# bentotten/radiation_ppo

Measured on AMD Instinct MI355X. Metric: env steps/sec (whole node) at 4096 envs; PPO iters/sec at 1/2/4/8 GPUs, higher is better.
Workload: dtype f32 policy / f64+int32 env

## Files before the change

### include/radsearch.h

```cpp
#ifndef RADSEARCH_H
#define RADSEARCH_H

#include <stddef.h>
#include <stdint.h>

#ifdef __cplusplus
extern "C" {
#endif

#define RS_ABI_VERSION 4
#define RS_OBS_DIM 11
#define RS_NUM_ACTIONS 9
#define RS_MAX_AGENTS 8
#define RS_MAX_OBS 7

typedef void* rs_stream_t;
typedef struct rs_handle rs_handle;

enum {
    RS_OK = 0,
    RS_ERR_INVALID_ARG = 1,
    RS_ERR_HIP = 2,
    RS_ERR_WORKSPACE = 3,
    RS_ERR_UNSUPPORTED = 4
// ... 55 lines not shown

int rs_poisson_probe(const double* lam, const uint32_t* t, const uint32_t* episode, const uint32_t* env_id, int64_t count, uint32_t seed,
                     int64_t* serial, int64_t* group3, int64_t* group4, int32_t* candidates, rs_stream_t stream);

int rs_error_flags(rs_handle* h, rs_stream_t stream, uint32_t* flags_out);

int rs_gae(const float* rew, const float* val, const uint8_t* cut, const float* last_val, float* adv, float* ret,
           int32_t T, int32_t M, double gamma, double lam, rs_stream_t stream);

size_t rs_ppo_prepare_workspace_bytes(int32_t N);
int rs_ppo_prepare(const uint8_t* cut, const float* adv, float* w, float* adv_n, float* mean_std, void* workspace, int32_t T, int32_t N,
                   int32_t n_total, rs_stream_t stream);

typedef struct rs_mlp_params {
    const float *w1, *b1, *w2, *b2, *w3, *b3;
} rs_mlp_params;

int rs_policy_forward(const rs_mlp_params* actor, const rs_mlp_params* critic, const float* x, int32_t M,
                      float* logits, float* value, rs_stream_t stream);

int rs_ff_team_step(const rs_mlp_params* actors, const rs_mlp_params* critics, int32_t num_agents, const float* x, const float* u,
                    int64_t* act, float* logp_val_boot, int8_t* act8, const uint8_t* mask, int32_t num_envs, rs_stream_t stream);

typedef struct rs_rollout_args {
    int32_t steps_per_epoch;
    int32_t steps_per_episode;
    float* obs;
    int64_t* act;
    float* logp;
    float* val;
    float* rew;
    float* last_val;
    uint8_t* cut;
    float* source_tar;
    float* cur_obs;
    double* w_count;
    double* w_mean;
    double* w_sq;
    double* w_std;
    int32_t* steps_in_ep;
    float* ep_ret;
    int32_t* done_count;
    int32_t* oob_count;
    double* ep_ret_sum;
    double* ep_len_sum;
    int32_t* ep_count;
    double* ep_ret_sq_sum;
    float* ep_ret_max;
    float* ep_ret_min;
} rs_rollout_args;

int rs_rollout(rs_handle* h, const rs_mlp_params* actor, const rs_mlp_params* critic, const rs_rollout_args* args,
               rs_stream_t stream);

typedef struct rs_ppo_batch {
    const float* x;
    const int64_t* act;
    const float* adv;
    const float* ret;
    const float* logp_old;
    const float* w;
    int32_t M;
    float clip_ratio, alpha, vf_coef;
} rs_ppo_batch;

size_t rs_ppo_grad_workspace_bytes(void);
#define RS_PPO_STATS_TAIL 16
#define RS_PPO_GRAD_FLOATS (10441 + RS_PPO_STATS_TAIL)
int rs_ppo_grad(const rs_mlp_params* actor, const rs_mlp_params* critic, const rs_ppo_batch* batch, float* grads,
                double* stats, void* workspace, const int32_t* stop_flag, rs_stream_t stream);

typedef struct rs_update_state {
    int32_t adam_step;
    int32_t stopped;
    int32_t iters;
    int32_t pad;
    double last_stats[5];
} rs_update_state;

int rs_adam_step(const rs_mlp_params* actor, const rs_mlp_params* critic, const float* grads, float* m, float* v,
                 const double* stats, rs_update_state* state, float lr, float kl_threshold, rs_stream_t stream);

int rs_ppo_update_step(const rs_mlp_params* actor, const rs_mlp_params* critic, const rs_ppo_batch* batch, float* grads,
                       double* stats, void* workspace, float* m, float* v, rs_update_state* state, float lr, float kl_threshold,
                       rs_stream_t stream);

typedef struct rs_maps rs_maps;
enum {
    RS_MAPERR_RING_FULL = 1,
    RS_MAPERR_VISIT_OVERFLOW = 2,
    RS_MAPERR_OFF_MAP = 4
};
size_t rs_maps_state_bytes(int32_t num_envs, int32_t num_agents, int32_t steps_per_episode, int32_t map_x, int32_t map_y);
int rs_maps_create(int32_t num_envs, int32_t num_agents, int32_t steps_per_episode, int32_t map_x, int32_t map_y,
                   double resolution_accuracy, const float* visit_table, void* workspace, size_t workspace_bytes,
                   rs_stream_t stream, rs_maps** out);
void rs_maps_destroy(rs_maps* m);
int rs_maps_reset(rs_maps* m, const uint8_t* mask, rs_stream_t stream);
int rs_maps_update(rs_maps* m, rs_handle* env, const float* obs, const float* pred, const uint8_t* mask, rs_stream_t stream);
int rs_maps_stack(rs_maps* m, float* actor_stack, float* critic_stack, rs_stream_t stream);
int rs_maps_field(rs_maps* m, const char* name, void** dev_ptr, int32_t* elem_bytes, int32_t* rows, int32_t* cols);

int32_t rs_cnn_trunk_slab_row(int32_t in_channels);
int32_t rs_cnn_trunk_slab_rows(int64_t num_samples, int32_t in_channels);
int32_t rs_cnn_trunk_scratch_floats(int32_t in_channels);
int rs_cnn_trunk_forward(const float* maps, const int64_t* cells, const int64_t* pcells, int32_t num_agents, int32_t agent,
// ... 259 lines not shown
```

### radiation_ppo_amd/_lib.py

```python
import ctypes as C
import os

import torch

_PKG = os.path.dirname(os.path.abspath(__file__))
LIB_PATH = os.environ.get("RS_LIB_PATH") or os.path.join(_PKG, "lib", "librs_hip.so")

RS_OBS_DIM = 11
RS_MAX_AGENTS = 8
RS_MAX_OBS = 7

ENVERR_ZERO_DIST = 1
ENVERR_IDLE_STALL = 2
ENVERR_CORRECT_CAP = 4
ENVERR_BAD_ACTION = 8
ENVERR_NO_PATH = 16

MAPERR_RING_FULL = 1
MAPERR_VISIT_OVERFLOW = 2
MAPERR_OFF_MAP = 4


class RsConfig(C.Structure):
    _fields_ = [
# ... 32 lines not shown
class RsMlpParams(C.Structure):
    _fields_ = [(n, C.c_void_p) for n in ("w1", "b1", "w2", "b2", "w3", "b3")]


class RsCnnHeadParams(C.Structure):
    _fields_ = [(n, C.c_void_p) for n in ("w1", "b1", "w2", "b2", "w3", "b3")]


class RsCnnConvParams(C.Structure):
    _fields_ = [(n, C.c_void_p) for n in ("w1", "b1", "w2", "b2")]


class RsRolloutArgs(C.Structure):
    _fields_ = [("steps_per_epoch", C.c_int32), ("steps_per_episode", C.c_int32)] + [
        (n, C.c_void_p) for n in ("obs", "act", "logp", "val", "rew", "last_val", "cut", "source_tar", "cur_obs", "w_count",
                                  "w_mean", "w_sq", "w_std", "steps_in_ep", "ep_ret", "done_count", "oob_count",
                                  "ep_ret_sum", "ep_len_sum", "ep_count", "ep_ret_sq_sum", "ep_ret_max", "ep_ret_min")]


class RsPpoBatch(C.Structure):
    _fields_ = [("x", C.c_void_p), ("act", C.c_void_p), ("adv", C.c_void_p), ("ret", C.c_void_p), ("logp_old", C.c_void_p),
                ("w", C.c_void_p), ("M", C.c_int32), ("clip_ratio", C.c_float), ("alpha", C.c_float), ("vf_coef", C.c_float)]


class RsInfo(C.Structure):
    _fields_ = [("out_of_bounds", C.c_void_p), ("out_of_bounds_count", C.c_void_p), ("blocked", C.c_void_p),
                ("collision", C.c_void_p)]


SYMBOLS = [
    ("rs_strerror", C.c_char_p, [C.c_int]),
    ("rs_abi_version", C.c_int, []),
    ("rs_state_bytes", C.c_size_t, [C.POINTER(RsConfig)]),
    ("rs_create", C.c_int, [C.POINTER(RsConfig), C.c_void_p, C.c_size_t, C.c_void_p, C.POINTER(C.c_void_p)]),
    ("rs_destroy", None, [C.c_void_p]),
    ("rs_state_field", C.c_int, [C.c_void_p, C.c_char_p, C.POINTER(C.c_void_p), C.POINTER(C.c_int32),
                                 C.POINTER(C.c_int32), C.POINTER(C.c_int32)]),
    ("rs_set_epoch_end", C.c_int, [C.c_void_p, C.c_void_p]),
    ("rs_reset", C.c_int, [C.c_void_p, C.c_void_p, C.c_void_p, C.c_void_p, C.c_void_p, C.c_void_p,
                           C.POINTER(RsInfo), C.c_void_p]),
    ("rs_refresh", C.c_int, [C.c_void_p, C.c_void_p, C.c_void_p, C.c_void_p, C.c_void_p, C.c_void_p, C.c_void_p, C.c_void_p,
                             C.c_void_p, C.c_void_p, C.c_void_p, C.c_void_p, C.POINTER(RsInfo), C.c_void_p]),
    ("rs_step", C.c_int, [C.c_void_p, C.c_void_p, C.c_void_p, C.c_void_p, C.c_void_p, C.c_void_p,
                          C.POINTER(RsInfo), C.c_void_p]),
    ("rs_action_uniforms", C.c_int, [C.c_void_p, C.c_void_p, C.c_void_p]),
    ("rs_poisson_probe", C.c_int, [C.c_void_p, C.c_void_p, C.c_void_p, C.c_void_p, C.c_int64, C.c_uint32, C.c_void_p, C.c_void_p,
                                   C.c_void_p, C.c_void_p, C.c_void_p]),
    ("rs_error_flags", C.c_int, [C.c_void_p, C.c_void_p, C.POINTER(C.c_uint32)]),
    ("rs_policy_forward", C.c_int, [C.POINTER(RsMlpParams), C.POINTER(RsMlpParams), C.c_void_p, C.c_int32, C.c_void_p,
                                    C.c_void_p, C.c_void_p]),
    ("rs_ff_team_step", C.c_int, [C.POINTER(RsMlpParams), C.POINTER(RsMlpParams), C.c_int32, C.c_void_p, C.c_void_p, C.c_void_p,
                                  C.c_void_p, C.c_void_p, C.c_void_p, C.c_int32, C.c_void_p]),
    ("rs_rollout", C.c_int, [C.c_void_p, C.POINTER(RsMlpParams), C.POINTER(RsMlpParams), C.POINTER(RsRolloutArgs), C.c_void_p]),
    ("rs_ppo_grad_workspace_bytes", C.c_size_t, []),
    ("rs_ppo_grad", C.c_int, [C.POINTER(RsMlpParams), C.POINTER(RsMlpParams), C.POINTER(RsPpoBatch), C.c_void_p, C.c_void_p,
                              C.c_void_p, C.c_void_p, C.c_void_p]),
    ("rs_adam_step", C.c_int, [C.POINTER(RsMlpParams), C.POINTER(RsMlpParams), C.c_void_p, C.c_void_p, C.c_void_p, C.c_void_p,
                               C.c_void_p, C.c_float, C.c_float, C.c_void_p]),
    ("rs_ppo_update_step", C.c_int, [C.POINTER(RsMlpParams), C.POINTER(RsMlpParams), C.POINTER(RsPpoBatch), C.c_void_p, C.c_void_p,
                                     C.c_void_p, C.c_void_p, C.c_void_p, C.c_void_p, C.c_float, C.c_float, C.c_void_p]),
    ("rs_maps_state_bytes", C.c_size_t, [C.c_int32, C.c_int32, C.c_int32, C.c_int32, C.c_int32]),
    ("rs_maps_create", C.c_int, [C.c_int32, C.c_int32, C.c_int32, C.c_int32, C.c_int32, C.c_double, C.c_void_p, C.c_void_p,
                                 C.c_size_t, C.c_void_p, C.POINTER(C.c_void_p)]),
    ("rs_maps_destroy", None, [C.c_void_p]),
    ("rs_maps_reset", C.c_int, [C.c_void_p, C.c_void_p, C.c_void_p]),
    ("rs_maps_update", C.c_int, [C.c_void_p, C.c_void_p, C.c_void_p, C.c_void_p, C.c_void_p, C.c_void_p]),
    ("rs_maps_stack", C.c_int, [C.c_void_p, C.c_void_p, C.c_void_p, C.c_void_p]),
    ("rs_maps_field", C.c_int, [C.c_void_p, C.c_char_p, C.POINTER(C.c_void_p), C.POINTER(C.c_int32), C.POINTER(C.c_int32),
                                C.POINTER(C.c_int32)]),
    ("rs_cnn_trunk_slab_row", C.c_int32, [C.c_int32]),
    ("rs_cnn_trunk_slab_rows", C.c_int32, [C.c_int64, C.c_int32]),
    ("rs_cnn_trunk_scratch_floats", C.c_int32, [C.c_int32]),
    ("rs_cnn_trunk_forward", C.c_int, [C.c_void_p, C.c_void_p, C.c_void_p, C.c_int32, C.c_int32, C.c_int64, C.c_void_p, C.c_void_p,
                                       C.c_void_p, C.c_void_p, C.c_void_p, C.c_void_p, C.c_void_p, C.c_void_p, C.c_void_p, C.c_void_p]),
    ("rs_cnn_trunk_backward", C.c_int, [C.c_void_p, C.c_void_p, C.c_void_p, C.c_int32, C.c_int32, C.c_int64, C.c_void_p, C.c_void_p,
                                        C.c_void_p, C.c_void_p, C.c_void_p, C.c_void_p, C.c_void_p, C.c_void_p]),
    ("rs_gae", C.c_int, [C.c_void_p, C.c_void_p, C.c_void_p, C.c_void_p, C.c_void_p, C.c_void_p, C.c_int32,
                         C.c_int32, C.c_double, C.c_double, C.c_void_p]),
    ("rs_ppo_prepare_workspace_bytes", C.c_size_t, [C.c_int32]),
    ("rs_ppo_prepare", C.c_int, [C.c_void_p] * 6 + [C.c_int32, C.c_int32, C.c_int32, C.c_void_p]),
    ("rs_pfgru_step", C.c_int, [C.c_void_p, C.c_void_p, C.c_void_p, C.c_void_p, C.c_void_p, C.c_void_p, C.c_void_p, C.c_void_p,
                                C.c_int32, C.c_double, C.c_void_p, C.c_int32, C.c_int32, C.c_void_p]),
    ("rs_pfgru_step_recorded", C.c_int, [C.c_void_p] * 7 + [C.c_int32, C.c_double, C.c_void_p, C.c_int32, C.c_int32, C.c_void_p]),
    ("rs_pfgru_pass", C.c_int, [C.c_void_p] * 7 + [C.c_double, C.c_void_p, C.c_void_p, C.c_int32, C.c_int32, C.c_void_p]),
    ("rs_pfgru_reset", C.c_int, [C.c_void_p, C.c_void_p, C.c_void_p, C.c_void_p, C.c_void_p, C.c_void_p, C.c_int32, C.c_int32,
                                 C.c_void_p]),
    ("rs_pfgru_sized_weight_floats", C.c_int32, [C.c_int32]),
    ("rs_pfgru_sized_step", C.c_int, [C.c_void_p] * 8 + [C.c_int32, C.c_double, C.c_void_p, C.c_int32, C.c_int32, C.c_int32, C.c_void_p]),
    ("rs_pfgru_sized_pass", C.c_int, [C.c_void_p] * 7 + [C.c_double, C.c_void_p, C.c_void_p, C.c_int32, C.c_int32, C.c_int32, C.c_void_p]),
    ("rs_pfgru_sized_step_recorded", C.c_int, [C.c_void_p] * 7 + [C.c_int32, C.c_double, C.c_void_p, C.c_int32, C.c_int32, C.c_int32,
                                                                    C.c_void_p]),
    ("rs_pfgru_sized_reset", C.c_int, [C.c_void_p] * 6 + [C.c_int32, C.c_int32, C.c_int32, C.c_void_p]),
    ("rs_pfgru_draws", C.c_int, [C.c_void_p, C.c_int32, C.c_int32, C.c_void_p, C.c_void_p, C.c_void_p, C.c_void_p]),
    ("rs_pfgru_train", C.c_int, [C.c_void_p] * 15 + [C.c_int32, C.c_int32, C.c_double, C.c_double, C.c_double, C.c_double, C.c_void_p]),
    ("rs_pfgru_train_keyed", C.c_int, [C.c_void_p] * 14 + [C.c_int32, C.c_int32, C.c_double, C.c_double, C.c_double, C.c_double, C.c_void_p]),
    ("rs_pfgru_sized_train_weight_floats", C.c_int32, [C.c_int32]),
    ("rs_pfgru_sized_train_grad_floats", C.c_int32, [C.c_int32]),
    ("rs_pfgru_sized_draws", C.c_int, [C.c_void_p, C.c_int32, C.c_int32, C.c_int32, C.c_void_p, C.c_void_p, C.c_void_p, C.c_void_p]),
    ("rs_pfgru_sized_train", C.c_int, [C.c_void_p] * 15 + [C.c_int32, C.c_int32, C.c_double, C.c_double, C.c_double, C.c_double, C.c_int32,
                                       C.c_void_p]),
    ("rs_rnn_policy_step", C.c_int, [C.c_void_p] * 10 + [C.c_int32, C.c_void_p]),
    ("rs_rnn_policy_step_rows", C.c_int, [C.c_void_p, C.c_void_p, C.c_int32, C.c_void_p, C.c_int32, C.c_void_p, C.c_void_p, C.c_int32, C.c_void_p,
                                          C.c_void_p, C.c_void_p, C.c_void_p, C.c_void_p, C.c_int32, C.c_void_p, C.c_int32, C.c_void_p]),
    ("rs_collect_pre", C.c_int, [C.POINTER(RsCollectState), C.c_void_p]),
    ("rs_collect_post_step", C.c_int, [C.POINTER(RsCollectState), C.c_int32, C.c_void_p]),
    ("rs_collect_post_reset", C.c_int, [C.POINTER(RsCollectState), C.c_int32, C.c_void_p]),
# ... 104 lines not shown
```

### radiation_ppo_amd/csrc/rs_ppo.hip

```cpp
#include <hip/hip_runtime.h>
#include <stdint.h>
#include <stdlib.h>
#include <string.h>

#include "../../include/radsearch.h"
#include "rs_mlp.hpp"
#include "rs_handle.hpp"

static inline RsMlpParams to_dev(const rs_mlp_params* p) { return RsMlpParams{p->w1, p->b1, p->w2, p->b2, p->w3, p->b3}; }

__device__ __forceinline__ void rs_exchange_x(const float (&xo)[RS_IN_PAD], float (&xp)[RS_IN_PAD]) {
#pragma unroll
    for (int k = 0; k < RS_IN_PAD; ++k) xp[k] = __shfl_xor(xo[k], 32);
}

__global__ void __launch_bounds__(64) rs_policy_forward_kernel(RsMlpParams pa, RsMlpParams pc, const float* __restrict__ x, int M,
                                                               float* __restrict__ logits, float* __restrict__ value) {
    extern __shared__ __align__(16) float smem_f[];
    RsMlpLds<8> A; RsMlpLds<1> Cn;
    A.carve(smem_f);
    Cn.carve(smem_f + rs_mlp_lds_floats(8));
    A.fill(pa); Cn.fill(pc);
    __syncthreads();
    const int lane = threadIdx.x & 63;
// ... 154 lines not shown
        }
        for (int q = 0; q < 5; ++q) spart[q][threadIdx.x] = t[q];
    }
    __syncthreads();
    if (threadIdx.x < 5) {
        double t = 0;
        for (int i = 0; i < 64; ++i) t += spart[threadIdx.x][i];
        stot[threadIdx.x] = t;
    }
    float g = 0.0f;
    if (grp == 0 && p < NA + NC) {
        g = part[0][col];
        for (int g2 = 1; g2 < 16; ++g2) g += part[g2][col];
        grads[p] = g;
    }
    __syncthreads();
    if (grp != 0) return;
    double t[5];
    for (int q = 0; q < 5; ++q) t[q] = stot[q];
    t[4] = -(t[4] - (double)vf * t[3] + (double)alpha * t[1]);
    const bool take = t[0] < (double)thr;
    if (take && p < NA + NC) {
        const int i = p;
        int seg = 0;
#pragma unroll
        for (int k = 1; k < 12; ++k) seg += (i >= S.off[k]) ? 1 : 0;
        float* pp = S.p[seg] + (i - S.off[seg]);
        const float b1 = 0.9f, b2 = 0.999f, eps = 1e-8f;
        const int step = adam_step + 1;
        const float mi = m[i] + (g - m[i]) * (1.0f - b1);
        const float vi = b2 * v[i] + (1.0f - b2) * g * g;
        m[i] = mi; v[i] = vi;
        const float bc1 = 1.0f - powf(b1, (float)step), bc2 = 1.0f - powf(b2, (float)step);
        const float step_size = lr / bc1;
        const float denom = sqrtf(vi) / sqrtf(bc2) + eps;
        *pp = *pp - step_size * (mi / denom);
    }
    if (blockIdx.x == 0 && threadIdx.x == 0) {
        for (int q = 0; q < 5; ++q) {
            stats[q] = t[q];
            const float hi = (float)t[q];
            grads[NA + NC + 2 * q] = hi;
            grads[NA + NC + 2 * q + 1] = (float)(t[q] - (double)hi);
            st->last_stats[q] = t[q];
        }
        for (int q = 10; q < RS_PPO_STATS_TAIL; ++q) grads[NA + NC + q] = 0.0f;
        st->iters += 1;
        if (take) st->adam_step = adam_step + 1; else st->stopped = 1;
    }
}

extern "C" {

int rs_rollout(rs_handle* h, const rs_mlp_params* actor, const rs_mlp_params* critic, const rs_rollout_args* args,
               rs_stream_t stream) {
    if (!h || !actor || !critic || !args) return RS_ERR_INVALID_ARG;
    const RsParams& P = h->P;
    if (P.A != 1 || (P.N % 16) != 0) return RS_ERR_UNSUPPORTED;
    const bool has_obs = P.obstruction_count != 0;
    if (has_obs && P.group != 1) return RS_ERR_UNSUPPORTED;
    if (args->steps_per_epoch < 1 || args->steps_per_episode < 1) return RS_ERR_INVALID_ARG;
    size_t lds = sizeof(float) * (size_t)(rs_mlp16_lds_floats(8) + rs_mlp16_lds_floats(1)) + 16;
    lds += (has_obs ? (2 * RS_MAX_VERT * RS_WAVE * 4 + RS_MAX_VERT * RS_WAVE * 8) : 0);
    lds += RS_WAVE * RS_OBS_DIM * 4 + RS_WAVE * 4 + 2 * RS_WAVE + rs_rollout16_mailbox_bytes();
    hipStream_t s = static_cast<hipStream_t>(stream);
    if (has_obs) hipLaunchKernelGGL(rs_rollout16_kernel<true>, dim3(P.N / 16), dim3(2 * RS_WAVE), lds, s, P, to_dev(actor), to_dev(critic), *args);
    else hipLaunchKernelGGL(rs_rollout16_kernel<false>, dim3(P.N / 16), dim3(2 * RS_WAVE), lds, s, P, to_dev(actor), to_dev(critic), *args);
    return hipGetLastError() == hipSuccess ? RS_OK : RS_ERR_HIP;
}

static_assert(sizeof(float) * rs_grad2_lds_floats(8) <= 160 * 1024 && sizeof(float) * rs_grad2_lds_floats(1) <= 160 * 1024,
              "K7 workgroup exceeds the CU's LDS");

size_t rs_ppo_grad_workspace_bytes(void) {
    const size_t slabs = RS_GRAD_BLOCKS;
    return slabs * (size_t)(rs_net_params(8) + rs_net_params(1)) * sizeof(float) + 2 * slabs * 5 * sizeof(double) + 1024;
}

static RsParamSeg rs_param_seg(const rs_mlp_params* actor, const rs_mlp_params* critic) {
    RsParamSeg S;
    const float* ptrs[12] = {actor->w1, actor->b1, actor->w2, actor->b2, actor->w3, actor->b3,
                             critic->w1, critic->b1, critic->w2, critic->b2, critic->w3, critic->b3};
    const int sizes[12] = {704, 64, 4096, 64, 512, 8, 704, 64, 4096, 64, 64, 1};
    int o = 0;
    for (int k = 0; k < 12; ++k) { S.p[k] = const_cast<float*>(ptrs[k]); S.off[k] = o; o += sizes[k]; }
    S.off[12] = o;
    return S;
}

int rs_adam_step(const rs_mlp_params* actor, const rs_mlp_params* critic, const float* grads, float* m, float* v,
                 const double* stats, rs_update_state* state, float lr, float kl_threshold, rs_stream_t stream) {
    if (!actor || !critic || !grads || !m || !v || !state) return RS_ERR_INVALID_ARG;
    const RsParamSeg S = rs_param_seg(actor, critic);
    const int o = S.off[12];
    hipStream_t s = static_cast<hipStream_t>(stream);
    hipLaunchKernelGGL(rs_adam_apply_kernel, dim3((o + 255) / 256), dim3(256), 0, s, S, grads, m, v, stats, state, lr, kl_threshold);
    hipLaunchKernelGGL(rs_adam_commit_kernel, dim3(1), dim3(1), 0, s, stats, grads + o, state, kl_threshold);
    return hipGetLastError() == hipSuccess ? RS_OK : RS_ERR_HIP;
}

struct RsGradWs { float *pa, *pc; double *sa, *sc; int* snap; };

static RsGradWs rs_grad_ws(void* workspace) {
    const int slabs = RS_GRAD_BLOCKS;
    RsGradWs w;
    w.pa = static_cast<float*>(workspace);
    w.pc = w.pa + (size_t)slabs * rs_net_params(8);
    w.sa = reinterpret_cast<double*>((reinterpret_cast<uintptr_t>(w.pc + (size_t)slabs * rs_net_params(1)) + 255) & ~uintptr_t(255));
    w.sc = w.sa + (size_t)slabs * 5;
    w.snap = reinterpret_cast<int*>(w.sc + (size_t)slabs * 5);
    return w;
}

static int rs_launch_k7(const rs_mlp_params* actor, const rs_mlp_params* critic, const rs_ppo_batch* batch, const RsGradWs& w,
                        const int32_t* stop_flag, const rs_update_state* ust, hipStream_t s, bool pair = false) {
    const size_t lds_a = sizeof(float) * (size_t)rs_grad2_lds_floats(8);
    const size_t lds_c = sizeof(float) * (size_t)rs_grad2_lds_floats(1);
    const size_t lds_p = lds_a > lds_c ? lds_a : lds_c;
    if (pair) {
        if (hipFuncSetAttribute(reinterpret_cast<const void*>(rs_ppo_grad2_pair_kernel), hipFuncAttributeMaxDynamicSharedMemorySize, (int)lds_p) != hipSuccess)
// ... 97 lines not shown
```

### radiation_ppo_amd/csrc/rs_rollout16.hpp

```cpp
#pragma once
#include "rs_mlp.hpp"

__host__ __device__ constexpr int rs_mlp16_lds_floats(int nout) { return 4 * 3 * 64 + 4 * 16 * 64 + 64 + 4 * nout * 16 + nout; }

template <int NOUT>
struct RsMlp16 {
    float* w1f;
    float* w2f;
    float* b2;
    float* w3g;
    float* b3;
    __device__ __forceinline__ void carve(float* base) {
        w1f = base; w2f = w1f + 4 * 3 * 64; b2 = w2f + 4 * 16 * 64; w3g = b2 + 64; b3 = w3g + 4 * NOUT * 16;
    }
    __device__ __forceinline__ void fill(const RsMlpParams& p) {
        const int tid = threadIdx.x, nt = blockDim.x;
        for (int i = tid; i < 4 * 3 * 64; i += nt) {
            const int l = i & 63, s = (i >> 6) % 3, it = i / (3 * 64);
            const int row = 16 * it + (l & 15), k = 4 * s + (l >> 4);
            w1f[i] = RS_TANH_PRESCALE * ((k < RS_IN) ? p.w1[row * RS_IN + k] : p.b1[row]);
        }
        for (int i = tid; i < 4 * 16 * 64; i += nt) {
            const int l = i & 63, ks = (i >> 6) & 15, it = i >> 10;
            const int unit = 16 * (ks >> 2) + 4 * (l >> 4) + (ks & 3);
// ... 18 lines not shown
#pragma unroll
            for (int ut = 0; ut < 4; ++ut) {
                const float4 wv = w[ut];
                w3[set][4 * ut + 0] = wv.x; w3[set][4 * ut + 1] = wv.y; w3[set][4 * ut + 2] = wv.z; w3[set][4 * ut + 3] = wv.w;
            }
        }
    }
    static __device__ __forceinline__ float park(float v) { float a; asm("v_accvgpr_write_b32 %0, %1" : "=a"(a) : "v"(v)); return a; }
    __device__ __forceinline__ void load(Regs& r) const {
        const int lane = threadIdx.x & 63, g = lane >> 4;
#pragma unroll
        for (int i = 0; i < 4 * 3; ++i) r.w1[i] = park(w1f[i * 64 + lane]);
#pragma unroll
        for (int i = 0; i < 4 * 16; ++i) r.w2[i] = park(w2f[i * 64 + lane]);
#pragma unroll
        for (int i = 0; i < 4 * 4; ++i) r.b2[i] = b2[16 * (i >> 2) + 4 * g + (i & 3)];
        if constexpr (NOUT == 8) {
            load_w3(r.w3);
#pragma unroll
            for (int i = 0; i < 32; ++i) r.w3[i >> 4][i & 15] = park(r.w3[i >> 4][i & 15]);
        }
    }
    template <bool REG>
    __device__ __forceinline__ void hidden(const float (&xs)[RS_IN_PAD], f32x4 (&H2)[4], const Regs& r) const {
        const int lane = threadIdx.x & 63, g = lane >> 4;
        f32x4 H1[4];
#pragma unroll
        for (int it = 0; it < 4; ++it)
#pragma unroll
            for (int q = 0; q < 4; ++q) { H1[it][q] = 0.0f; H2[it][q] = REG ? r.b2[4 * it + q] : b2[16 * it + 4 * g + q]; }
#pragma unroll
        for (int s = 0; s < 3; ++s) {
            const float b = (g == 0) ? xs[4 * s] : (g == 1) ? xs[4 * s + 1] : (g == 2) ? xs[4 * s + 2] : xs[4 * s + 3];
#pragma unroll
            for (int it = 0; it < 4; ++it)
                H1[it] = __builtin_amdgcn_mfma_f32_16x16x4f32(REG ? r.w1[it * 3 + s] : w1f[(it * 3 + s) * 64 + lane], b, H1[it], 0, 0, 0);
        }
#pragma unroll
        for (int it = 0; it < 4; ++it)
#pragma unroll
            for (int q = 0; q < 4; ++q) H1[it][q] = rs_tanh_scaled(H1[it][q]);
#pragma unroll
        for (int ks = 0; ks < 16; ++ks) {
            const float b = H1[ks >> 2][ks & 3];
#pragma unroll
            for (int it = 0; it < 4; ++it)
                H2[it] = __builtin_amdgcn_mfma_f32_16x16x4f32(REG ? r.w2[it * 16 + ks] : w2f[(it * 16 + ks) * 64 + lane], b, H2[it], 0, 0, 0);
        }
#pragma unroll
        for (int it = 0; it < 4; ++it)
#pragma unroll
            for (int q = 0; q < 4; ++q) H2[it][q] = rs_tanh_scaled(H2[it][q]);
    }
    __device__ __forceinline__ float combine(float p, int o) const {
        const int g = (threadIdx.x & 63) >> 4;
        const float q1 = __shfl_xor(p, 16);
        const float s01 = (g & 1) ? (q1 + p) : (p + q1);
        const float q2 = __shfl_xor(s01, 32);
        return ((g & 2) ? (q2 + s01) : (s01 + q2)) + b3[o];
    }
    __device__ __forceinline__ void output(const f32x4 (&H2)[4], float (&out)[NOUT]) const {
        const int g = (threadIdx.x & 63) >> 4;
#pragma unroll
        for (int o = 0; o < NOUT; ++o) {
            const float4* w = reinterpret_cast<const float4*>(w3g + (g * NOUT + o) * 16);
            float p = 0.0f;
#pragma unroll
            for (int ut = 0; ut < 4; ++ut) {
                const float4 wv = w[ut];
                p = fmaf(wv.x, H2[ut][0], p); p = fmaf(wv.y, H2[ut][1], p);
                p = fmaf(wv.z, H2[ut][2], p); p = fmaf(wv.w, H2[ut][3], p);
            }
            out[o] = combine(p, o);
        }
    }
    __device__ __forceinline__ void output_mfma(const f32x4 (&H2)[4], float (&out)[NOUT], const float (&w3)[2][16]) const {
        static_assert(NOUT == 8, "two chains of four outputs");
        f32x4 pacc[2];
#pragma unroll
        for (int i = 0; i < 4; ++i) { pacc[0][i] = 0.0f; pacc[1][i] = 0.0f; }
#pragma unroll
        for (int ut = 0; ut < 4; ++ut)
#pragma unroll
            for (int q = 0; q < 4; ++q) {
                pacc[0] = __builtin_amdgcn_mfma_f32_4x4x1f32(w3[0][4 * ut + q], H2[ut][q], pacc[0], 0, 0, 0);
                pacc[1] = __builtin_amdgcn_mfma_f32_4x4x1f32(w3[1][4 * ut + q], H2[ut][q], pacc[1], 0, 0, 0);
            }
#pragma unroll
        for (int o = 0; o < NOUT; ++o) out[o] = combine(pacc[o >> 2][o & 3], o);
    }
    __device__ __forceinline__ void forward(const float (&xs)[RS_IN_PAD], float (&out)[NOUT]) const {
        f32x4 H2[4];
        Regs none;
        hidden<false>(xs, H2, none);
        output(H2, out);
    }
};

__device__ __forceinline__ void rs_bcast_x16(const float (&xo)[RS_IN_PAD], float (&xs)[RS_IN_PAD]) {
    const int src = threadIdx.x & 15;
#pragma unroll
    for (int k = 0; k < RS_IN_PAD; ++k) xs[k] = __shfl(xo[k], src);
}

constexpr int RS_MB_PRE = 0, RS_MB_POST = 16 * RS_IN_PAD, RS_MB_FLAGS = 2 * 16 * RS_IN_PAD, RS_MB_SLOT = 2 * 16 * RS_IN_PAD + 16;
__host__ __device__ constexpr int rs_rollout16_mailbox_bytes() { return 2 * RS_MB_SLOT * 4; }

#ifdef RS_K6_PARENT_CHAIN
constexpr bool RS_K6_SHORT = false;
#else
constexpr bool RS_K6_SHORT = true;
#endif
#ifdef RS_K6_SERIAL_DRAW
constexpr bool RS_K6_GROUP = false;
#else
constexpr bool RS_K6_GROUP = true;
#endif
#ifndef RS_K6_OBS_BY_WAVE1
#define RS_K6_OBS_BY_WAVE1 true
#endif
template <bool HAS_OBS> struct RsK6Cfg {
    static constexpr bool reg_weights = RS_K6_SHORT && !HAS_OBS;
    static constexpr bool mfma_out = RS_K6_SHORT;
    static constexpr bool reg_state = RS_K6_SHORT;
    static constexpr bool group_draw = RS_K6_GROUP && reg_state;
    static constexpr bool obs_by_wave1 = RS_K6_SHORT && RS_K6_GROUP && RS_K6_OBS_BY_WAVE1 && !HAS_OBS;
};

#ifdef RS_K6_STAMPS
#define RS_K6_NPH 16
__device__ unsigned long long rs_k6_stamp_table[2][RS_K6_NPH];
__device__ __forceinline__ unsigned long long rs_k6_now() {
    unsigned long long t;
    asm volatile("s_memtime %0\n\ts_waitcnt lgkmcnt(0)" : "=s"(t) :: "memory");
    return t;
}
#define RS_K6STAMP_DECL unsigned long long k6_acc[RS_K6_NPH] = {0}; const unsigned long long k6_rt0 = __builtin_amdgcn_s_memrealtime(); \
                        unsigned long long k6_last = rs_k6_now(); unsigned long long k6p[3] = {0, 0, 0};
#define RS_K6STAMP(i) do { __builtin_amdgcn_sched_barrier(0); const unsigned long long t_ = rs_k6_now(); k6_acc[i] += t_ - k6_last; k6_last = t_; \
                           __builtin_amdgcn_sched_barrier(0); } while (0)
#define RS_K6STAMP_TRIPS(active) do { const int m_ = rs_k6p_wave_max((active) ? (int)k6p[1] : 0); k6_acc[9] += m_; k6_acc[10] += m_ > 3 ? m_ - 3 : 0; } while (0)
#define RS_K6STAMP_PHILOX(t0) do { k6_acc[12] += rs_k6p_now() - (t0); } while (0)
#define RS_K6STAMP_EXIT(tmpl, steps) do { if ((threadIdx.x & 63) == 0) { k6_acc[8] = k6p[0]; k6_acc[11] = k6p[2]; k6_acc[14] = __builtin_amdgcn_s_memrealtime() - k6_rt0; k6_acc[15] = (steps); \
                           for (int q = 0; q < RS_K6_NPH; ++q) atomicAdd(&rs_k6_stamp_table[tmpl][q], k6_acc[q]); } } while (0)
#else
#define RS_K6STAMP_DECL
#define RS_K6STAMP(i) do {} while (0)
#define RS_K6STAMP_TRIPS(active) do {} while (0)
#define RS_K6STAMP_PHILOX(t0) do {} while (0)
#define RS_K6STAMP_EXIT(tmpl, steps) do {} while (0)
#endif

template <bool HAS_OBS>
__global__ void __launch_bounds__(128) rs_rollout16_kernel(RsParams P, RsMlpParams pa, RsMlpParams pc, rs_rollout_args R) {
    extern __shared__ __align__(16) unsigned char smem[];
    float* wts = reinterpret_cast<float*>(smem);
    unsigned char* p = smem + sizeof(float) * (size_t)(rs_mlp16_lds_floats(8) + rs_mlp16_lds_floats(1));
    p = reinterpret_cast<unsigned char*>((reinterpret_cast<uintptr_t>(p) + 15) & ~uintptr_t(15));
    int* lds_geo = reinterpret_cast<int*>(p);
    uint32_t* lds_adj = reinterpret_cast<uint32_t*>(p + RS_MAX_VERT * RS_WAVE * 4);
    double* lds_d = reinterpret_cast<double*>(p + 2 * RS_MAX_VERT * RS_WAVE * 4);
    float* tile = reinterpret_cast<float*>(p + (HAS_OBS ? (2 * RS_MAX_VERT * RS_WAVE * 4 + RS_MAX_VERT * RS_WAVE * 8) : 0));
    float* lds_rew = tile + RS_WAVE * RS_OBS_DIM;
    uint8_t* lds_done = reinterpret_cast<uint8_t*>(lds_rew + RS_WAVE);
    uint8_t* lds_oob = lds_done + RS_WAVE;
    float* mbox = reinterpret_cast<float*>(lds_oob + RS_WAVE);

    RsMlp16<8> ACT; RsMlp16<1> CRT;
    ACT.carve(wts);
    CRT.carve(wts + rs_mlp16_lds_floats(8));
    ACT.fill(pa); CRT.fill(pc);

    const int wave = __builtin_amdgcn_readfirstlane((int)(threadIdx.x >> 6));
    const int lane = threadIdx.x & 63, j = lane & 15;
    const bool own = lane < 16;
    const int n = blockIdx.x * 16 + j;
    const int N = P.N, T = R.steps_per_epoch, L = R.steps_per_episode;
    const int cj = lane >> 4;
    RsGeo g{lds_geo, 0, 0, 0};
    if (HAS_OBS && wave == 0) {
        rs_load_geo(P, n, own, lds_geo, g);
        g.off = __shfl(g.off, j); g.stride = __shfl(g.stride, j); g.n = __shfl(g.n, j);
    }
    __syncthreads();

    if (wave == 1) {
        for (int t = -1; t < T; ++t) {
            __syncthreads();
            const float* M = mbox + (t & 1) * RS_MB_SLOT;
            if constexpr (RsK6Cfg<HAS_OBS>::obs_by_wave1) {
                if (t + 1 < T) {
                    float* dst = R.obs + ((size_t)(t + 1) * N + (size_t)blockIdx.x * 16) * RS_OBS_DIM;
                    const int* F = reinterpret_cast<const int*>(M + RS_MB_FLAGS);
                    for (int i = lane; i < 16 * RS_OBS_DIM; i += RS_WAVE) {
                        const int e = i / RS_OBS_DIM, k = i - e * RS_OBS_DIM;
                        dst[i] = M[((F[e] & 1) ? RS_MB_POST : RS_MB_PRE) + e * RS_IN_PAD + k];
                    }
                }
            }
            float xs[RS_IN_PAD];
#pragma unroll
            for (int k = 0; k < RS_IN_PAD; ++k) xs[k] = M[RS_MB_PRE + j * RS_IN_PAD + k];
            float vb;
            { float vv[1]; CRT.forward(xs, vv); vb = vv[0]; }
            const int fl = reinterpret_cast<const int*>(M + RS_MB_FLAGS)[j];
            const bool cut = (fl & 1) != 0, boot = (fl & 2) != 0;
            float v = vb;
            if (__ballot(cut) != 0ull) {
#pragma unroll
                for (int k = 0; k < RS_IN_PAD; ++k) xs[k] = M[RS_MB_POST + j * RS_IN_PAD + k];
                float vv[1];
                CRT.forward(xs, vv);
                v = cut ? vv[0] : vb;
            }
            if (own) {
                if (t >= 0) R.last_val[(size_t)t * N + n] = (cut && boot) ? vb : 0.0f;
                if (t + 1 < T) R.val[(size_t)(t + 1) * N + n] = v;
            }
        }
        return;
    }

    float oraw[RS_OBS_DIM];
#pragma unroll
    for (int k = 0; k < RS_OBS_DIM; ++k) oraw[k] = R.cur_obs[(size_t)n * RS_OBS_DIM + k];
    RsWelford W{R.w_count[n], R.w_mean[n], R.w_sq[n], R.w_std[n]};
    int steps = R.steps_in_ep[n];
    float ep_ret = R.ep_ret[n];
    int done_count = 0, oob_count = 0, ep_count = 0;
    double ep_ret_sum = 0.0, ep_len_sum = 0.0, ep_ret_sq = 0.0;
    float ep_ret_max = -INFINITY, ep_ret_min = INFINITY;
    const uint32_t k0 = P.seed, k1 = P.env_id_base + (uint32_t)n;
    using Cfg = RsK6Cfg<HAS_OBS>;
    RsEnvRegs E;
    RsAgentRegs S;
    E.load(P, n);
    S.load(P, (size_t)n);
    RsMlp16<8>::Regs AR;
    if constexpr (Cfg::reg_weights) ACT.load(AR);

    float xo[RS_IN_PAD], xs[RS_IN_PAD];
#pragma unroll
    for (int k = 0; k < RS_OBS_DIM; ++k) xo[k] = oraw[k];
    xo[0] = W.standardize(oraw[0]);
    xo[11] = 1.0f;
    rs_bcast_x16(xo, xs);
    {
        float* M = mbox + RS_MB_SLOT;
        if (own) {
#pragma unroll
            for (int k = 0; k < RS_IN_PAD; ++k) M[RS_MB_PRE + j * RS_IN_PAD + k] = xo[k];
            reinterpret_cast<int*>(M + RS_MB_FLAGS)[j] = 0;
        }
    }
    __syncthreads();

    RsOut O;
    O.obs_row = tile + j * RS_OBS_DIM;
    O.reward = lds_rew + j - (size_t)n;
    O.team = nullptr;
    O.done = lds_done + j - (size_t)n;
    O.oob = lds_oob + j - (size_t)n;
    O.oobc = nullptr; O.blocked = nullptr; O.collision = nullptr;

    RS_K6STAMP_DECL
    for (int t = 0; t < T; ++t) {
        const size_t row = (size_t)t * N + n;
        float* M = mbox + (t & 1) * RS_MB_SLOT;
        float lg[8];
        u32x4 ph{0u, 0u, 0u, 0u};
        if constexpr (Cfg::group_draw) {
#ifdef RS_K6_STAMPS
            const unsigned long long p0 = rs_k6p_now();
#endif
            ph = philox4x32_10(cj ? (uint32_t)(cj - 1) : 0u, E.tstep, E.episode, cj ? RS_STREAM_STEP : RS_STREAM_ACT, k0, k1);
            RS_K6STAMP_PHILOX(p0);
            RS_K6STAMP(13);
        }
        {
            f32x4 H2[4];
            ACT.template hidden<Cfg::reg_weights>(xs, H2, AR);
            RS_K6STAMP(0);
            if constexpr (!Cfg::mfma_out) ACT.output(H2, lg);
            else if constexpr (Cfg::reg_weights) ACT.output_mfma(H2, lg, AR.w3);
            else { float w3[2][16]; ACT.load_w3(w3); ACT.output_mfma(H2, lg, w3); }
            RS_K6STAMP(1);
        }
        int a = 0;
        float logp = 0.0f;
        if (own) {
            float mx = lg[0];
#pragma unroll
            for (int q = 1; q < 8; ++q) mx = fmaxf(mx, lg[q]);
            float se = 0.0f;
#pragma unroll
            for (int q = 0; q < 8; ++q) se += __expf(lg[q] - mx);
            const float lse = __logf(se);
            if constexpr (!Cfg::group_draw) {
#ifdef RS_K6_STAMPS
                const unsigned long long p0 = rs_k6p_now();
#endif
                ph = philox4x32_10(0u, E.tstep, E.episode, RS_STREAM_ACT, k0, k1);
                RS_K6STAMP_PHILOX(p0);
            }
            const float u = (float)(ph.x >> 8) * (1.0f / 16777216.0f);
            float cdf = 0.0f;
#pragma unroll
            for (int q = 0; q < 8; ++q) {
                const float lpq = (lg[q] - mx) - lse;
                cdf += __expf(lpq);
                if (q < 7) a += (cdf <= u) ? 1 : 0;
            }
#pragma unroll
            for (int q = 0; q < 8; ++q) logp = (a == q) ? ((lg[q] - mx) - lse) : logp;
            if constexpr (!Cfg::obs_by_wave1) {
#pragma unroll
                for (int k = 0; k < RS_OBS_DIM; ++k) tile[lane * RS_OBS_DIM + k] = xo[k];
            }
        }
        __builtin_amdgcn_wave_barrier();
        RS_K6STAMP(2);
        if constexpr (!Cfg::obs_by_wave1) {
            float* dst = R.obs + ((size_t)t * N + (size_t)blockIdx.x * 16) * RS_OBS_DIM;
            for (int i = lane; i < 16 * RS_OBS_DIM; i += RS_WAVE) dst[i] = tile[i];
        }
        __builtin_amdgcn_wave_barrier();
        bool cut = false;
        bool over = false, boot = false, ended = t == T - 1;
        if (own) {
            R.act[row] = (int64_t)a;
            R.logp[row] = logp;
            R.source_tar[row * 2 + 0] = (float)E.sx;
            R.source_tar[row * 2 + 1] = (float)E.sy;
        }
        RS_K6STAMP(3);
// ... 41 lines not shown
            if (over) {
                ep_ret_sum += (double)ep_ret; ep_len_sum += (double)steps; ep_count += 1;
                ep_ret_sq += (double)ep_ret * (double)ep_ret;
                ep_ret_max = fmaxf(ep_ret_max, ep_ret); ep_ret_min = fminf(ep_ret_min, ep_ret);
            }
        }
        RS_K6STAMP(5);
        if (HAS_OBS ? (__shfl((int)cut, j) != 0) : cut) {
            if (ended) P.epoch_end[n] = 1;
            if constexpr (Cfg::reg_state) { S.store(P, (size_t)n); E.store(P, n); }
            if constexpr (HAS_OBS) rs_env_reset_lane<true, 4>(P, g, n, lds_geo, lds_adj, lds_d, tile + j * RS_OBS_DIM, O, j, cj);
            else rs_env_reset_lane<false>(P, g, n, lds_geo, lds_adj, lds_d, tile + lane * RS_OBS_DIM, O);
            E.load(P, n);
            if constexpr (Cfg::reg_state) S.load(P, (size_t)n);
        }
        if constexpr (Cfg::group_draw && !HAS_OBS) {
            if (__ballot(cut) != 0ull) { E.from_lane(j); S.from_lane(j); }
        }
        if (own) {
            if (cut) {
                W.reset();
#pragma unroll
                for (int k = 0; k < RS_OBS_DIM; ++k) oraw[k] = tile[lane * RS_OBS_DIM + k];
                W.update((double)oraw[0]);
#pragma unroll
                for (int k = 1; k < RS_OBS_DIM; ++k) xo[k] = oraw[k];
                xo[0] = W.standardize(oraw[0]);
                steps = 0;
                ep_ret = 0.0f;
#pragma unroll
                for (int k = 0; k < RS_IN_PAD; ++k) M[RS_MB_POST + j * RS_IN_PAD + k] = xo[k];
            }
        }
        RS_K6STAMP(6);
        rs_bcast_x16(xo, xs);
        __syncthreads();
        RS_K6STAMP(7);
    }
    RS_K6STAMP_EXIT(HAS_OBS ? 1 : 0, (unsigned long long)T);
    if constexpr (Cfg::reg_state) {
        if (HAS_OBS || own) { S.store(P, (size_t)n); E.store(P, n); }
    }
    if (own) {
#pragma unroll
        for (int k = 0; k < RS_OBS_DIM; ++k) R.cur_obs[(size_t)n * RS_OBS_DIM + k] = oraw[k];
        R.w_count[n] = W.count; R.w_mean[n] = W.mean; R.w_sq[n] = W.sq; R.w_std[n] = W.std;
        R.steps_in_ep[n] = steps;
        R.ep_ret[n] = ep_ret;
        R.done_count[n] = done_count; R.oob_count[n] = oob_count; R.ep_count[n] = ep_count;
        R.ep_ret_sum[n] = ep_ret_sum; R.ep_len_sum[n] = ep_len_sum;
        R.ep_ret_sq_sum[n] = ep_ret_sq; R.ep_ret_max[n] = ep_ret_max; R.ep_ret_min[n] = ep_ret_min;
    }
}
```

Before: 44.21 million.

## Split actor hidden layers across four waves with LDS exchange in rollout kernel

Adds a tiled mode for the no-obstruction rollout kernel in which the actor's two hidden layers are divided across four waves. Each wave keeps its slice of the layer weights in registers and runs MFMA on it, then the waves exchange activations through new LDS buffers, with barriers between the layers. The goal is to shorten the serial per-step MLP latency when there are few blocks, i.e. when the grid is at most one block per CU. Larger grids fall back to the original two-wave kernel. The cost is extra __syncthreads and LDS traffic on every step, plus a larger block.

Measured after the change: 44.90 million, median of 6. +1.6%, better.

```diff
diff --git a/include/radsearch.h b/include/radsearch.h
--- a/include/radsearch.h
+++ b/include/radsearch.h
@@ -131,6 +131,7 @@
 
 int rs_rollout(rs_handle* h, const rs_mlp_params* actor, const rs_mlp_params* critic, const rs_rollout_args* args,
                rs_stream_t stream);
+size_t rs_rollout_lds_bytes(int has_obs);
 
 typedef struct rs_ppo_batch {
     const float* x;
diff --git a/radiation_ppo_amd/_lib.py b/radiation_ppo_amd/_lib.py
--- a/radiation_ppo_amd/_lib.py
+++ b/radiation_ppo_amd/_lib.py
@@ -108,6 +108,7 @@
     ("rs_ff_team_step", C.c_int, [C.POINTER(RsMlpParams), C.POINTER(RsMlpParams), C.c_int32, C.c_void_p, C.c_void_p, C.c_void_p,
                                   C.c_void_p, C.c_void_p, C.c_void_p, C.c_int32, C.c_void_p]),
     ("rs_rollout", C.c_int, [C.c_void_p, C.POINTER(RsMlpParams), C.POINTER(RsMlpParams), C.POINTER(RsRolloutArgs), C.c_void_p]),
+    ("rs_rollout_lds_bytes", C.c_size_t, [C.c_int]),
     ("rs_ppo_grad_workspace_bytes", C.c_size_t, []),
     ("rs_ppo_grad", C.c_int, [C.POINTER(RsMlpParams), C.POINTER(RsMlpParams), C.POINTER(RsPpoBatch), C.c_void_p, C.c_void_p,
                               C.c_void_p, C.c_void_p, C.c_void_p]),
diff --git a/radiation_ppo_amd/csrc/rs_ppo.hip b/radiation_ppo_amd/csrc/rs_ppo.hip
--- a/radiation_ppo_amd/csrc/rs_ppo.hip
+++ b/radiation_ppo_amd/csrc/rs_ppo.hip
@@ -230,6 +230,14 @@
 
 extern "C" {
 
+size_t rs_rollout_lds_bytes(int has_obs) {
+    size_t lds = sizeof(float) * (size_t)(rs_mlp16_lds_floats(8) + rs_mlp16_lds_floats(1)) + 16;
+    lds += (has_obs ? (2 * RS_MAX_VERT * RS_WAVE * 4 + RS_MAX_VERT * RS_WAVE * 8) : 0);
+    lds += RS_WAVE * RS_OBS_DIM * 4 + RS_WAVE * 4 + 2 * RS_WAVE + rs_rollout16_mailbox_bytes();
+    lds += has_obs ? rs_rollout16_exchange_bytes<true>() : rs_rollout16_exchange_bytes<false>();
+    return lds;
+}
+
 int rs_rollout(rs_handle* h, const rs_mlp_params* actor, const rs_mlp_params* critic, const rs_rollout_args* args,
                rs_stream_t stream) {
     if (!h || !actor || !critic || !args) return RS_ERR_INVALID_ARG;
@@ -238,12 +246,16 @@
     const bool has_obs = P.obstruction_count != 0;
     if (has_obs && P.group != 1) return RS_ERR_UNSUPPORTED;
     if (args->steps_per_epoch < 1 || args->steps_per_episode < 1) return RS_ERR_INVALID_ARG;
-    size_t lds = sizeof(float) * (size_t)(rs_mlp16_lds_floats(8) + rs_mlp16_lds_floats(1)) + 16;
-    lds += (has_obs ? (2 * RS_MAX_VERT * RS_WAVE * 4 + RS_MAX_VERT * RS_WAVE * 8) : 0);
-    lds += RS_WAVE * RS_OBS_DIM * 4 + RS_WAVE * 4 + 2 * RS_WAVE + rs_rollout16_mailbox_bytes();
+    const size_t lds = rs_rollout_lds_bytes(has_obs ? 1 : 0);
     hipStream_t s = static_cast<hipStream_t>(stream);
-    if (has_obs) hipLaunchKernelGGL(rs_rollout16_kernel<true>, dim3(P.N / 16), dim3(2 * RS_WAVE), lds, s, P, to_dev(actor), to_dev(critic), *args);
-    else hipLaunchKernelGGL(rs_rollout16_kernel<false>, dim3(P.N / 16), dim3(2 * RS_WAVE), lds, s, P, to_dev(actor), to_dev(critic), *args);
+    static int cus = 0;
+    if (cus == 0) {
+        int dev = 0, n = 0;
+        cus = (hipGetDevice(&dev) == hipSuccess && hipDeviceGetAttribute(&n, hipDeviceAttributeMultiprocessorCount, dev) == hipSuccess && n > 0) ? n : 256;
+    }
+    if (has_obs) hipLaunchKernelGGL(rs_rollout16_kernel<true>, dim3(P.N / 16), dim3(RsK6Cfg<true>::waves * RS_WAVE), lds, s, P, to_dev(actor), to_dev(critic), *args);
+    else if (P.N / 16 <= cus) hipLaunchKernelGGL(rs_rollout16_kernel<false>, dim3(P.N / 16), dim3(RsK6Cfg<false>::waves * RS_WAVE), lds, s, P, to_dev(actor), to_dev(critic), *args);
+    else hipLaunchKernelGGL(rs_rollout16_wide_kernel, dim3(P.N / 16), dim3(2 * RS_WAVE), lds, s, P, to_dev(actor), to_dev(critic), *args);
     return hipGetLastError() == hipSuccess ? RS_OK : RS_ERR_HIP;
 }
 
diff --git a/radiation_ppo_amd/csrc/rs_rollout16.hpp b/radiation_ppo_amd/csrc/rs_rollout16.hpp
--- a/radiation_ppo_amd/csrc/rs_rollout16.hpp
+++ b/radiation_ppo_amd/csrc/rs_rollout16.hpp
@@ -94,6 +94,49 @@
 #pragma unroll
             for (int q = 0; q < 4; ++q) H2[it][q] = rs_tanh_scaled(H2[it][q]);
     }
+    template <int NT> struct TileRegs { float w1[NT * 3], w2[NT * 16], b2[NT * 4]; };
+    template <int NT>
+    __device__ __forceinline__ void load_tiles(TileRegs<NT>& r, int it0) const {
+        const int lane = threadIdx.x & 63, g = lane >> 4;
+#pragma unroll
+        for (int i = 0; i < NT * 3; ++i) r.w1[i] = park(w1f[(it0 * 3 + i) * 64 + lane]);
+#pragma unroll
+        for (int i = 0; i < NT * 16; ++i) r.w2[i] = park(w2f[(it0 * 16 + i) * 64 + lane]);
+#pragma unroll
+        for (int i = 0; i < NT * 4; ++i) r.b2[i] = b2[16 * (it0 + (i >> 2)) + 4 * g + (i & 3)];
+    }
+    template <int NT>
+    __device__ __forceinline__ void tile_layer1(const float (&b)[3], const TileRegs<NT>& r, f32x4 (&H1)[NT]) const {
+#pragma unroll
+        for (int n = 0; n < NT; ++n)
+#pragma unroll
+            for (int q = 0; q < 4; ++q) H1[n][q] = 0.0f;
+#pragma unroll
+        for (int s = 0; s < 3; ++s)
+#pragma unroll
+            for (int n = 0; n < NT; ++n) H1[n] = __builtin_amdgcn_mfma_f32_16x16x4f32(r.w1[n * 3 + s], b[s], H1[n], 0, 0, 0);
+#pragma unroll
+        for (int n = 0; n < NT; ++n)
+#pragma unroll
+            for (int q = 0; q < 4; ++q) H1[n][q] = rs_tanh_scaled(H1[n][q]);
+    }
+    template <int NT>
+    __device__ __forceinline__ void tile_layer2(const f32x4 (&H1)[4], const TileRegs<NT>& r, f32x4 (&H2)[NT]) const {
+#pragma unroll
+        for (int n = 0; n < NT; ++n)
+#pragma unroll
+            for (int q = 0; q < 4; ++q) H2[n][q] = r.b2[4 * n + q];
+#pragma unroll
+        for (int ks = 0; ks < 16; ++ks) {
+            const float b = H1[ks >> 2][ks & 3];
+#pragma unroll
+            for (int n = 0; n < NT; ++n) H2[n] = __builtin_amdgcn_mfma_f32_16x16x4f32(r.w2[n * 16 + ks], b, H2[n], 0, 0, 0);
+        }
+#pragma unroll
+        for (int n = 0; n < NT; ++n)
+#pragma unroll
+            for (int q = 0; q < 4; ++q) H2[n][q] = rs_tanh_scaled(H2[n][q]);
+    }
     __device__ __forceinline__ float combine(float p, int o) const {
         const int g = (threadIdx.x & 63) >> 4;
         const float q1 = __shfl_xor(p, 16);
@@ -161,7 +204,19 @@
 #ifndef RS_K6_OBS_BY_WAVE1
 #define RS_K6_OBS_BY_WAVE1 true
 #endif
-template <bool HAS_OBS> struct RsK6Cfg {
+#ifndef RS_K6_TILE_WAVES
+#define RS_K6_TILE_WAVES 4
+#endif
+static_assert(RS_K6_TILE_WAVES == 0 || RS_K6_TILE_WAVES == 2 || RS_K6_TILE_WAVES == 4, "RS_K6_TILE_WAVES: 0, 2 or 4");
+#ifndef RS_K6_TILE_WAVES_OBS
+#define RS_K6_TILE_WAVES_OBS 0
+#endif
+static_assert(RS_K6_TILE_WAVES_OBS == 0 || RS_K6_TILE_WAVES_OBS == 2 || RS_K6_TILE_WAVES_OBS == 4, "RS_K6_TILE_WAVES_OBS: 0, 2 or 4");
+template <bool HAS_OBS> constexpr int rs_k6_tile_waves = (RS_K6_SHORT && RS_K6_GROUP && RS_K6_OBS_BY_WAVE1) ? (HAS_OBS ? RS_K6_TILE_WAVES_OBS : RS_K6_TILE_WAVES) : 0;
+template <bool HAS_OBS, int TW = rs_k6_tile_waves<HAS_OBS>> struct RsK6Cfg {
+    static constexpr int tile_waves = TW;
+    static constexpr int tiles_per_wave = tile_waves ? 4 / tile_waves : 4;
+    static constexpr int waves = tile_waves ? 4 : 2;
     static constexpr bool reg_weights = RS_K6_SHORT && !HAS_OBS;
     static constexpr bool mfma_out = RS_K6_SHORT;
     static constexpr bool reg_state = RS_K6_SHORT;
@@ -169,8 +224,11 @@
     static constexpr bool obs_by_wave1 = RS_K6_SHORT && RS_K6_GROUP && RS_K6_OBS_BY_WAVE1 && !HAS_OBS;
 };
 
+template <bool HAS_OBS> __host__ __device__ constexpr int rs_rollout16_exchange_bytes() { return RsK6Cfg<HAS_OBS>::tile_waves ? 2 * 4 * 64 * 16 : 0; }
+static_assert(rs_rollout16_mailbox_bytes() % 16 == 0 && (RS_WAVE * RS_OBS_DIM * 4 + RS_WAVE * 4 + 2 * RS_WAVE) % 16 == 0, "exchange arrays: 16-byte aligned");
+
 #ifdef RS_K6_STAMPS
-#define RS_K6_NPH 16
+#define RS_K6_NPH 20
 __device__ unsigned long long rs_k6_stamp_table[2][RS_K6_NPH];
 __device__ __forceinline__ unsigned long long rs_k6_now() {
     unsigned long long t;
@@ -193,8 +251,8 @@
 #define RS_K6STAMP_EXIT(tmpl, steps) do {} while (0)
 #endif
 
-template <bool HAS_OBS>
-__global__ void __launch_bounds__(128) rs_rollout16_kernel(RsParams P, RsMlpParams pa, RsMlpParams pc, rs_rollout_args R) {
+template <bool HAS_OBS, int TW>
+__device__ __forceinline__ void rs_rollout16_body(const RsParams& P, const RsMlpParams& pa, const RsMlpParams& pc, const rs_rollout_args& R) {
     extern __shared__ __align__(16) unsigned char smem[];
     float* wts = reinterpret_cast<float*>(smem);
     unsigned char* p = smem + sizeof(float) * (size_t)(rs_mlp16_lds_floats(8) + rs_mlp16_lds_floats(1));
@@ -207,6 +265,8 @@
     uint8_t* lds_done = reinterpret_cast<uint8_t*>(lds_rew + RS_WAVE);
     uint8_t* lds_oob = lds_done + RS_WAVE;
     float* mbox = reinterpret_cast<float*>(lds_oob + RS_WAVE);
+    f32x4* xch1 = reinterpret_cast<f32x4*>(mbox + 2 * RS_MB_SLOT);
+    f32x4* xch2 = xch1 + 4 * RS_WAVE;
 
     RsMlp16<8> ACT; RsMlp16<1> CRT;
     ACT.carve(wts);
@@ -226,11 +286,42 @@
     }
     __syncthreads();
 
-    if (wave == 1) {
+    using Cfg = RsK6Cfg<HAS_OBS, TW>;
+    constexpr int NT = Cfg::tiles_per_wave;
+    const int it0 = Cfg::tile_waves == 4 ? (wave == 0 ? 0 : wave == 1 ? 3 : wave - 1) : (wave == 3 ? 2 : 0);
+    const bool tiler = Cfg::tile_waves == 4 || (Cfg::tile_waves == 2 && wave >= 2);
+    typename RsMlp16<8>::template TileRegs<NT> TR;
+    if constexpr (Cfg::tile_waves != 0) {
+        if (tiler) ACT.template load_tiles<NT>(TR, it0);
+    }
+
+    if (wave != 0) {
         for (int t = -1; t < T; ++t) {
             __syncthreads();
             const float* M = mbox + (t & 1) * RS_MB_SLOT;
-            if constexpr (RsK6Cfg<HAS_OBS>::obs_by_wave1) {
+            if constexpr (Cfg::tile_waves != 0) {
+                if (t + 1 < T) {
+                    f32x4 H1[4], Ht[NT];
+                    if (tiler) {
+                        const float* x = M + ((reinterpret_cast<const int*>(M + RS_MB_FLAGS)[j] & 1) ? RS_MB_POST : RS_MB_PRE) + j * RS_IN_PAD + cj;
+                        const float b[3] = {x[0], x[4], x[8]};
+                        ACT.template tile_layer1<NT>(b, TR, Ht);
+#pragma unroll
+                        for (int i = 0; i < NT; ++i) xch1[(it0 + i) * RS_WAVE + lane] = Ht[i];
+                    }
+                    __syncthreads();
+                    if (tiler) {
+#pragma unroll
+                        for (int i = 0; i < 4; ++i) H1[i] = xch1[i * RS_WAVE + lane];
+                        ACT.template tile_layer2<NT>(H1, TR, Ht);
+#pragma unroll
+                        for (int i = 0; i < NT; ++i) xch2[(it0 + i) * RS_WAVE + lane] = Ht[i];
+                    }
+                    __syncthreads();
+                }
+                if (wave != 1) continue;
+            }
+            if constexpr (Cfg::obs_by_wave1) {
                 if (t + 1 < T) {
                     float* dst = R.obs + ((size_t)(t + 1) * N + (size_t)blockIdx.x * 16) * RS_OBS_DIM;
                     const int* F = reinterpret_cast<const int*>(M + RS_MB_FLAGS);
@@ -273,13 +364,16 @@
     double ep_ret_sum = 0.0, ep_len_sum = 0.0, ep_ret_sq = 0.0;
     float ep_ret_max = -INFINITY, ep_ret_min = INFINITY;
     const uint32_t k0 = P.seed, k1 = P.env_id_base + (uint32_t)n;
-    using Cfg = RsK6Cfg<HAS_OBS>;
     RsEnvRegs E;
     RsAgentRegs S;
     E.load(P, n);
     S.load(P, (size_t)n);
     RsMlp16<8>::Regs AR;
-    if constexpr (Cfg::reg_weights) ACT.load(AR);
+    if constexpr (Cfg::tile_waves != 0 && Cfg::reg_weights) {
+        ACT.load_w3(AR.w3);
+#pragma unroll
+        for (int i = 0; i < 32; ++i) AR.w3[i >> 4][i & 15] = RsMlp16<8>::park(AR.w3[i >> 4][i & 15]);
+    } else if constexpr (Cfg::reg_weights) ACT.load(AR);
 
     float xo[RS_IN_PAD], xs[RS_IN_PAD];
 #pragma unroll
@@ -321,8 +415,37 @@
         }
         {
             f32x4 H2[4];
-            ACT.template hidden<Cfg::reg_weights>(xs, H2, AR);
-            RS_K6STAMP(0);
+            if constexpr (Cfg::tile_waves != 0) {
+                if constexpr (Cfg::tile_waves == 4) {
+                    f32x4 Ht[NT];
+                    const float b[3] = {(cj == 0) ? xs[0] : (cj == 1) ? xs[1] : (cj == 2) ? xs[2] : xs[3],
+                                        (cj == 0) ? xs[4] : (cj == 1) ? xs[5] : (cj == 2) ? xs[6] : xs[7],
+                                        (cj == 0) ? xs[8] : (cj == 1) ? xs[9] : (cj == 2) ? xs[10] : xs[11]};
+                    ACT.template tile_layer1<NT>(b, TR, Ht);
+                    xch1[it0 * RS_WAVE + lane] = Ht[0];
+                    RS_K6STAMP(0);
+                    __syncthreads();
+                    f32x4 H1[4];
+#pragma unroll
+                    for (int i = 0; i < 4; ++i) H1[i] = xch1[i * RS_WAVE + lane];
+                    RS_K6STAMP(16);
+                    ACT.template tile_layer2<NT>(H1, TR, Ht);
+                    xch2[it0 * RS_WAVE + lane] = Ht[0];
+                    RS_K6STAMP(0);
+                    __syncthreads();
+                } else {
+                    RS_K6STAMP(0);
+                    __syncthreads();
+                    RS_K6STAMP(16);
+                    __syncthreads();
+                }
+#pragma unroll
+                for (int i = 0; i < 4; ++i) H2[i] = xch2[i * RS_WAVE + lane];
+                RS_K6STAMP(17);
+            } else {
+                ACT.template hidden<Cfg::reg_weights>(xs, H2, AR);
+                RS_K6STAMP(0);
+            }
             if constexpr (!Cfg::mfma_out) ACT.output(H2, lg);
             else if constexpr (Cfg::reg_weights) ACT.output_mfma(H2, lg, AR.w3);
             else { float w3[2][16]; ACT.load_w3(w3); ACT.output_mfma(H2, lg, w3); }
@@ -470,3 +593,11 @@
         R.ep_ret_sq_sum[n] = ep_ret_sq; R.ep_ret_max[n] = ep_ret_max; R.ep_ret_min[n] = ep_ret_min;
     }
 }
+
+template <bool HAS_OBS>
+__global__ void __launch_bounds__(RsK6Cfg<HAS_OBS>::waves * RS_WAVE) rs_rollout16_kernel(RsParams P, RsMlpParams pa, RsMlpParams pc, rs_rollout_args R) {
+    rs_rollout16_body<HAS_OBS, RsK6Cfg<HAS_OBS>::tile_waves>(P, pa, pc, R);
+}
+__global__ void __launch_bounds__(2 * RS_WAVE) rs_rollout16_wide_kernel(RsParams P, RsMlpParams pa, RsMlpParams pc, rs_rollout_args R) {
+    rs_rollout16_body<false, 0>(P, pa, pc, R);
+}
```
